# limix/CellRegMap

Hardware: AMD Instinct MI355X
Metric: variant-tests/sec (interaction test) (higher is better)
Workload: dtype f64

## Files before the change

### cellregmap_amd/csrc/api_core.hip

```cpp
#include <dlfcn.h>

#include <algorithm>
#include <atomic>
#include <cstdarg>
#include <mutex>

#include <map>

#include "crm_internal.h"
#include "eigh.h"

namespace crm {

static thread_local std::string g_error;

void set_error(const char* fmt, ...) {
    char buf[1024];
    va_list ap;
    va_start(ap, fmt);
    vsnprintf(buf, sizeof buf, fmt, ap);
    va_end(ap);
    g_error = buf;
}

// ... 235 lines not shown

int crm_set_null_fit_polish(crm_ctx* c, int on) {
    return crm::guarded_on("crm_set_null_fit_polish", c, [&]() -> int {
    if (!c) return CRM_ERR_ARG;
    c->polish = on != 0;
    return CRM_OK;
    });
}

int crm_set_progress_callback(crm_ctx* c, void (*callback)(long, long, void*), void* user) {
    return crm::guarded_on("crm_set_progress_callback", c, [&]() -> int {
    if (!c) return CRM_ERR_ARG;
    if (callback) c->progress[std::this_thread::get_id()] = crm_ctx::Progress{callback, user};
    else c->progress.erase(std::this_thread::get_id());
    return CRM_OK;
    });
}

int crm_set_fast_rotation(crm_ctx* c, int on) {
    return crm::guarded_on("crm_set_fast_rotation", c, [&]() -> int {
    if (!c) return CRM_ERR_ARG;
    c->fast_T = on != 0;
    return CRM_OK;
    });
}

extern "C++" {
namespace crm {
namespace {
struct FormSlot { const char* name; int value; bool set; };
FormSlot g_forms[] = {{"gram_staged", 0, false}, {"kr_no_tail", 0, false}, {"nullfit_per_wave", 0, false}, {"kin_fold", 0, false},
                      {"eigh_one_stage", 0, false}, {"nullfit_exact", 0, false}, {"donor_pairs", 0, false},
                      {"pairs_without_kinship_term", 0, false}, {"flat_kappa_milli", 0, false}, {"chase_abort", 0, false}, {"nullfit_one_per_wave", 0, false},
                      {"kin_diag", 0, false}, {"donor_pairs_rotate", 0, false}};
std::mutex g_forms_mu;
}
int form(const char* name, int otherwise) {
    std::lock_guard<std::mutex> lock(g_forms_mu);
    for (const FormSlot& f : g_forms)
        if (strcmp(f.name, name) == 0) return f.set ? f.value : otherwise;
    return otherwise;
}
}
}

int crm_test_set_form(const char* name, int value, int reset) {
    return crm::guarded("crm_test_set_form", [&]() -> int {
    if (!name) return CRM_ERR_ARG;
    std::lock_guard<std::mutex> lock(crm::g_forms_mu);
    for (crm::FormSlot& f : crm::g_forms)
        if (strcmp(f.name, name) == 0) {
            f.value = value;
            f.set = reset == 0;
            return CRM_OK;
        }
    crm::set_error("crm_test_set_form: no kernel form is called '%s'", name);
    return CRM_ERR_ARG;
    });
}

int crm_kernel_timer_reset(crm_ctx* c) {
    return crm::guarded_on("crm_kernel_timer_reset", c, [&]() -> int {
    if (!c) return CRM_ERR_ARG;
    CRM_HIP(hipSetDevice(c->device));
    CRM_HIP(hipStreamSynchronize(c->stream));
    c->timed_used = 0;
    c->kr_flops = 0.0;
// ... 270 lines not shown
```

### cellregmap_amd/csrc/blockops.hip

```cpp
#include "nullfit.h"

namespace crm {

namespace {

constexpr int STAT_SPLITS = 64;

__device__ __forceinline__ void row_and_chunk(int chunks, long& row, int& chunk) {
    row = blockIdx.x / (unsigned)chunks;
    chunk = (int)(blockIdx.x - (unsigned)row * (unsigned)chunks);
}
inline dim3 row_chunk_grid(long rows, int chunks) { return dim3((unsigned)(rows * chunks)); }

template <int C>
__global__ __launch_bounds__(256) void variant_stats_kernel(const double* __restrict__ G, long ldg,
                                                           long cells, int variants,
                                                           const double* __restrict__ y,
                                                           const double* __restrict__ W, long ldw,
                                                           double* __restrict__ partial) {
    __shared__ double red[4][C + 2][64];
    const int tx = threadIdx.x & 63, ty = threadIdx.x >> 6;
    const int b = blockIdx.x * 64 + tx;
    const long per = (cells + STAT_SPLITS - 1) / STAT_SPLITS;
    const long i0 = (long)blockIdx.y * per;
// ... 449 lines not shown
}

__global__ void pair_rows_sym_kernel(const double* __restrict__ C, long ldc, int variants, int k0, double* __restrict__ S,
                                     long lds) {
    const int a = blockIdx.y;
    const long e = (long)blockIdx.x * blockDim.x + threadIdx.x;
    if (e >= (long)variants * k0) return;
    const long b = e / k0;
    const int i = (int)(e - b * k0);
    const int lo = a < i ? a : i, hi = a < i ? i : a;
    const long pidx = (long)lo * k0 - (long)lo * (lo - 1) / 2 + (hi - lo);
    S[(long)a * lds + e] = C[b * ldc + pidx];
}

int launch_pair_rows_sym(hipStream_t st, const double* C, long ldc, int variants, int k0, double* S, long lds) {
    if (variants <= 0 || k0 <= 0) return CRM_OK;
    dim3 grid((unsigned)(((long)variants * k0 + 255) / 256), (unsigned)k0);
    hipLaunchKernelGGL(pair_rows_sym_kernel, grid, dim3(256), 0, st, C, ldc, variants, k0, S, lds);
    CRM_HIP(hipGetLastError());
    return CRM_OK;
}

constexpr int DP_VARIANTS = 4, DP_MAX_SLOTS = 32;

template <int DP_SLOTS>
__global__ __launch_bounds__(256) void donor_pairs_expand_kernel(const double* __restrict__ P, long p_slab, long ldp, int donors,
                                                                  int variants, int k0, int k1, double* __restrict__ S, long lds,
                                                                  double* __restrict__ Psum, long psum_slab, long row_d, long row_j) {
    extern __shared__ double tile[];
    const int npair = k0 * (k0 + 1) / 2, total = DP_VARIANTS * npair;
    const int v0 = blockIdx.x * DP_VARIANTS, tid = threadIdx.x;
    const int per = (donors + gridDim.y - 1) / gridDim.y;
    const int d0 = blockIdx.y * per, d1 = min(donors, d0 + per);
    if (d0 >= d1) return;
    double acc[DP_SLOTS], x[DP_SLOTS];
    int src[DP_SLOTS];
#pragma unroll
    for (int q = 0; q < DP_SLOTS; q++) {
        const int e = tid + 256 * q, v = e / npair, pr = e - v * npair;
        acc[q] = 0.0;
        src[q] = e < total && v0 + v < variants ? (int)((long)(v0 + v) * ldp + pr) : -1;
    }
    auto fetch = [&](int d) {
        const double* __restrict__ Pd = P + (size_t)d * p_slab;
#pragma unroll
        for (int q = 0; q < DP_SLOTS; q++)
            if (tid + 256 * q < total) x[q] = src[q] >= 0 ? Pd[src[q]] : 0.0;
    };
    const int row_len = DP_VARIANTS * k0;
    const int vw = tid / k0, iw = tid - vw * k0;
    const bool writer = tid < row_len && v0 + vw < variants;
    const int base_i = iw * k0 - iw * (iw - 1) / 2 - iw;
    const double* __restrict__ mine = tile + vw * npair;
    fetch(d0);
    for (int d = d0; d < d1; d++) {
#pragma unroll
        for (int q = 0; q < DP_SLOTS; q++)
            if (tid + 256 * q < total) { acc[q] += x[q]; tile[tid + 256 * q] = x[q]; }
        __syncthreads();
        if (d + 1 < d1) fetch(d + 1);
        if (writer) {
            double* __restrict__ Sd = S + (size_t)(k1 + (long)d * row_d) * lds + (long)v0 * k0 + tid;
            for (int j = 0; j < k0; j++) {
                const int pidx = j <= iw ? j * k0 - j * (j - 1) / 2 + (iw - j) : base_i + j;
                Sd[(long)j * row_j * lds] = mine[pidx];
            }
        }
// ... 1 lines not shown
    }
    double* __restrict__ out = Psum + (size_t)blockIdx.y * psum_slab;
#pragma unroll
    for (int q = 0; q < DP_SLOTS; q++)
        if (tid + 256 * q < total && src[q] >= 0) out[src[q]] = acc[q];
}

bool donor_pairs_serves(int k0) { return k0 >= 2 && DP_VARIANTS * (k0 * (k0 + 1) / 2) <= 256 * DP_MAX_SLOTS && DP_VARIANTS * k0 <= 256; }

int launch_donor_pairs_expand(hipStream_t st, const double* P, long p_slab, long ldp, int donors, int variants, int k0, int k1,
                              double* S, long lds, double* Psum, long psum_slab, int splits, long row_d, long row_j) {
    if (row_d <= 0) { row_d = k0; row_j = 1; }
    if (variants <= 0 || donors <= 0) return CRM_OK;
    if (!donor_pairs_serves(k0) || splits < 1) {
        set_error("donor pairs: k0=%d outside the supported range", k0);
        return CRM_ERR_UNSUPPORTED;
    }
    const size_t lds_bytes = sizeof(double) * DP_VARIANTS * (size_t)(k0 * (k0 + 1) / 2);
    dim3 grid((unsigned)((variants + DP_VARIANTS - 1) / DP_VARIANTS), (unsigned)splits);
    const int slots = (DP_VARIANTS * (k0 * (k0 + 1) / 2) + 255) / 256;
#define CRM_DP_LAUNCH(SL)                                                                                                        \
    hipLaunchKernelGGL(donor_pairs_expand_kernel<SL>, grid, dim3(256), lds_bytes, st, P, p_slab, ldp, donors, variants, k0, k1, \
                       S, lds, Psum, psum_slab, row_d, row_j)
    if (slots <= 4) CRM_DP_LAUNCH(4);
    else if (slots <= 8) CRM_DP_LAUNCH(8);
    else if (slots <= 16) CRM_DP_LAUNCH(16);
    else if (slots <= 24) CRM_DP_LAUNCH(24);
    else CRM_DP_LAUNCH(32);
#undef CRM_DP_LAUNCH
    CRM_HIP(hipGetLastError());
    return CRM_OK;
}

constexpr int DR_LDU = 80;
typedef double v4d __attribute__((ext_vector_type(4)));

__device__ __forceinline__ void lds_barrier() { asm volatile("s_waitcnt lgkmcnt(0)\n\ts_barrier" ::: "memory"); }

template <int DP_SLOTS>
__global__ __launch_bounds__(256, 2) void donor_pairs_rotate_kernel(const double* __restrict__ P, long p_slab, long ldp, int donors,
                                                                     int variants, int k0, const double* __restrict__ U, long u_slab,
                                                                     long ldu, double* __restrict__ A, long lda,
                                                                     double* __restrict__ Psum, long psum_slab) {
    extern __shared__ __align__(16) double smem[];
    const int npair = k0 * (k0 + 1) / 2, total = DP_VARIANTS * npair;
    const int KS = (k0 + 3) / 4, JT = (k0 + 15) / 16, urows = 4 * KS;
    double* const tile = smem;
    double* const ut = smem + ((total + 1) & ~1);
    const int v0 = blockIdx.x * DP_VARIANTS, tid = threadIdx.x;
    const int per = (donors + gridDim.y - 1) / gridDim.y;
    const int d0 = blockIdx.y * per, d1 = min(donors, d0 + per);
    if (d0 >= d1) return;
    double acc[DP_SLOTS];
#pragma unroll
    for (int q = 0; q < DP_SLOTS; q++) acc[q] = 0.0;
    const float inv_npair = 1.0f / (float)npair;
    const int vmax = min(DP_VARIANTS, variants - v0);
    auto src_of = [&](int q) __attribute__((always_inline)) -> int {
        int e = tid + 256 * q;
        asm volatile("" : "+v"(e));
        int v = (int)((float)e * inv_npair);
        v = v * npair > e ? v - 1 : ((v + 1) * npair <= e ? v + 1 : v);
        return e < total && v < vmax ? v * (int)ldp + (e - v * npair) : -1;
    };
    const int lane = tid & 63, l15 = lane & 15, lq = lane >> 4;
    const int w = __builtin_amdgcn_readfirstlane(tid >> 6);
    const int i = 16 * w + l15;
    int pidx[16];
#pragma unroll
    for (int ks = 0; ks < 16; ks++) {
        const int k = 4 * ks + lq, lo = k < i ? k : i, hi = k < i ? i : k;
        pidx[ks] = k < k0 && i < k0 ? lo * k0 - lo * (lo - 1) / 2 + (hi - lo) : 0;
    }
    for (int d = d0; d < d1; d++) {
        const double* __restrict__ Pd = P + (size_t)d * p_slab + (long)v0 * ldp;
#pragma unroll
        for (int q0 = 0; q0 < DP_SLOTS; q0 += 8) {
            double x[8];
            int sq[8];
#pragma unroll
            for (int q = 0; q < 8; q++) sq[q] = src_of(q0 + q);
#pragma unroll
            for (int q = 0; q < 8; q++) x[q] = Pd[sq[q] >= 0 ? sq[q] : 0];
#pragma unroll
            for (int q = 0; q < 8; q++)
                if (tid + 256 * (q0 + q) < total) {
                    const double xv = sq[q] >= 0 ? x[q] : 0.0;
                    acc[q0 + q] += xv;
                    tile[tid + 256 * (q0 + q)] = xv;
                }
        }
        const double* __restrict__ Ud = U + (size_t)d * u_slab + (tid & 63);
        double* __restrict__ ud = ut + (tid >> 6) * DR_LDU + (tid & 63);
#pragma unroll
        for (int q0 = 0; q0 < 16; q0 += 8) {
            double u[8];
#pragma unroll
            for (int q = 0; q < 8; q++) {
                int r = min((tid >> 6) + 4 * (q0 + q), urows - 1);
                asm volatile("" : "+v"(r));
                u[q] = Ud[(long)r * ldu];
            }
#pragma unroll
            for (int q = 0; q < 8; q++)
                if ((tid >> 6) + 4 * (q0 + q) < urows) ud[4 * (q0 + q) * DR_LDU] = u[q];
        }
        lds_barrier();
        if (w < JT) {
            for (int b = 0; b < DP_VARIANTS && v0 + b < variants; b++) {
                unsigned uo = (unsigned)(lq * DR_LDU + l15);
                asm volatile("" : "+v"(uo));
                const double* __restrict__ ub = ut + uo;
                const double* __restrict__ pb = tile + b * npair;
                v4d c[4];
#pragma unroll
                for (int t = 0; t < 4; t++) c[t] = (v4d){0.0, 0.0, 0.0, 0.0};
                double a[2], bf[2][4];
                auto frag = [&](int ks, int slot) __attribute__((always_inline)) {
                    a[slot] = pb[pidx[ks]];
#pragma unroll
                    for (int t = 0; t < 4; t++)
                        if (t < JT) bf[slot][t] = ub[4 * ks * DR_LDU + 16 * t];
                };
                frag(0, 0);
#pragma unroll
                for (int ks = 0; ks < 16; ks++) {
                    if (ks < KS) {
                        if (ks + 1 < KS) frag(ks + 1, (ks + 1) & 1);
#pragma unroll
                        for (int t = 0; t < 4; t++)
                            if (t < JT) c[t] = __builtin_amdgcn_mfma_f64_16x16x4f64(a[ks & 1], bf[ks & 1][t], c[t], 0, 0, 0);
                        __builtin_amdgcn_sched_barrier(0);
                    }
                }
                double* __restrict__ Ab = A + (size_t)((long)(v0 + b) * k0) * lda + (long)d * k0;
#pragma unroll
                for (int reg = 0; reg < 4; reg++) {
                    int r = 16 * w + lq + 4 * reg;
                    asm volatile("" : "+v"(r));
                    if (r < k0) {
#pragma unroll
                        for (int t = 0; t < 4; t++) {
                            const int j = 16 * t + l15;
                            if (t < JT && j < k0) Ab[(long)r * lda + j] = c[t][reg];
                        }
                    }
                }
            }
        }
        lds_barrier();
    }
    double* __restrict__ out = Psum + (size_t)blockIdx.y * psum_slab + (long)v0 * ldp;
#pragma unroll
    for (int q = 0; q < DP_SLOTS; q++) {
        const int sq = src_of(q);
        if (sq >= 0) out[sq] = acc[q];
    }
}

bool donor_pairs_rotate_serves(int k0) { return donor_pairs_serves(k0) && DP_VARIANTS * (k0 * (k0 + 1) / 2) <= 256 * 24; }

int launch_donor_pairs_rotate(hipStream_t st, const double* P, long p_slab, long ldp, int donors, int variants, int k0,
                              const double* U, long u_slab, long ldu, int k2pad, double* A, long lda, double* Psum, long psum_slab,
                              int splits) {
    if (variants <= 0 || donors <= 0) return CRM_OK;
    if (!donor_pairs_rotate_serves(k0) || splits < 1 || k2pad < 4 * ((k0 + 3) / 4) || ldu < 64) {
        set_error("donor pairs rotation: k0=%d / k2pad=%d outside the supported range", k0, k2pad);
        return CRM_ERR_UNSUPPORTED;
    }
    const int total = DP_VARIANTS * (k0 * (k0 + 1) / 2);
    const size_t lds_bytes = sizeof(double) * ((size_t)((total + 1) & ~1) + (size_t)4 * ((k0 + 3) / 4) * DR_LDU);
    dim3 grid((unsigned)((variants + DP_VARIANTS - 1) / DP_VARIANTS), (unsigned)splits);
    const int slots = (total + 255) / 256;
#define CRM_DR_LAUNCH(SL)                                                                                                         \
    do {                                                                                                                          \
        CRM_HIP(hipFuncSetAttribute(reinterpret_cast<const void*>(&donor_pairs_rotate_kernel<SL>),                                \
                                    hipFuncAttributeMaxDynamicSharedMemorySize, (int)lds_bytes));                                 \
        hipLaunchKernelGGL(donor_pairs_rotate_kernel<SL>, grid, dim3(256), lds_bytes, st, P, p_slab, ldp, donors, variants, k0, \
                           U, u_slab, ldu, A, lda, Psum, psum_slab);                                                              \
    } while (0)
    if (slots <= 8) CRM_DR_LAUNCH(8);
    else if (slots <= 16) CRM_DR_LAUNCH(16);
    else CRM_DR_LAUNCH(24);
#undef CRM_DR_LAUNCH
    CRM_HIP(hipGetLastError());
    return CRM_OK;
}

__global__ void scale_rows_kernel(const double* __restrict__ src, long ld_src, const double* __restrict__ scale, long ld_scale,
                                  int cols, double* __restrict__ dst, long ld_dst) {
    const long k = blockIdx.x;
    const double f = scale[k * ld_scale];
    for (int j = threadIdx.x; j < cols; j += blockDim.x) dst[k * ld_dst + j] = src[k * ld_src + j] * f;
}

int launch_scale_rows(hipStream_t st, const double* src, long ld_src, const double* scale, long ld_scale, long rows, int cols,
                      double* dst, long ld_dst) {
    if (rows <= 0 || cols <= 0) return CRM_OK;
    hipLaunchKernelGGL(scale_rows_kernel, dim3((unsigned)rows), dim3(128), 0, st, src, ld_src, scale, ld_scale, cols, dst, ld_dst);
    CRM_HIP(hipGetLastError());
    return CRM_OK;
}

__global__ void pair_rows_kernel(const double* __restrict__ C, long ldc, int variants, int k1, int k0,
                                 double* __restrict__ S, long lds) {
    const int a = blockIdx.y;
    const long e = (long)blockIdx.x * blockDim.x + threadIdx.x;
    if (e >= (long)variants * k0) return;
    const long b = e / k0;
    const int i = (int)(e - b * k0);
    S[(long)a * lds + e] = C[b * ldc + (long)a * k0 + i];
}

int launch_pair_rows(hipStream_t st, const double* C, long ldc, int variants, int k1, int k0, double* S, long lds) {
    if (variants <= 0 || k1 <= 0) return CRM_OK;
    dim3 grid((unsigned)(((long)variants * k0 + 255) / 256), (unsigned)k1);
// ... 64 lines not shown
```

### cellregmap_amd/csrc/nullfit.h

```cpp
#pragma once
#include "crm_internal.h"

namespace crm {

struct NullFitRho {
    const double* T;
    const double* ty;
    const double* tW;
    const double* S0;
    long ldT, ldW;
    int r;
    int pad_;
};

struct NullFitTrial {
    double lml, delta, scale;
    int use_g, nfev;
    double margin;
    double noise;
    double curv;
};

struct NullFitOut {
    int rho_index;
// ... 55 lines not shown
                         const double* y, const double* W, long ldw, int c, double* partial,
                         double* gg, double* gy, double* gW, long ld_gW);
size_t variant_stats_workspace(int variants, int c);
int launch_ortho_block(hipStream_t st, const double* G, long ldg, long cells_pad, int variants, int cols,
                       const double* W, long ldw, int c, const double* proj, const double* gW, long ld_gW,
                       double* coef, long ld_coef, double* thr, double* Gx, long ldx);
int launch_ortho_rank(hipStream_t st, const double* gg, const double* thr, int variants, int* drop);
int launch_collinear_flag(hipStream_t st, const double* gg, const double* gW, long ld_gW, const double* proj, int c,
                          int variants, double tau, int* near);
int launch_gather_block(hipStream_t st, const double* src, long ld_src, long cells_pad, long cells,
                        const int* row_index, const int* col_index, int variants, double* dst,
                        long ld_dst, int dst_cols);
int launch_gather_slabs(hipStream_t st, const double* src, long ld_src, long rows, const int* ord, int npairs,
                        int k0, double* dst, long ld_dst, int dst_cols);
int launch_gather_rows(hipStream_t st, const double* src, long ld_src, const int* map, long rows, int cols, double* dst,
                       long ld_dst);
int launch_kin_operand(hipStream_t st, const double* U, int k2, const double* H, long ldh, int k1, const int* map, long rows,
                       double* Y, long ldy);
int launch_kin_verify(hipStream_t st, const double* H, long ldh, int k1, const double* U, int k2, const int* group,
                      const double* hKd, long ldk, long m, long n, unsigned long long* out);
int launch_kin_sum_e1(hipStream_t st, const double* S, long ld_s, int KT, int k2, int k1, int groups, long cols, double* AH,
                      long ld_ah);
int launch_pair_features(hipStream_t st, const double* H, long ldh, int k1, const double* Ep, long ld_ep, int k0,
                         long cells_pad, double* P, long ldp);
int launch_pair_rows(hipStream_t st, const double* C, long ldc, int variants, int k1, int k0, double* S, long lds);
int launch_same_columns(hipStream_t st, const double* H, long ldh, const double* Ep, long ld_ep, long cells, int k, int* flag);
int launch_pair_rows_sym(hipStream_t st, const double* C, long ldc, int variants, int k0, double* S, long lds);
bool donor_pairs_serves(int k0);
int launch_donor_pairs_expand(hipStream_t st, const double* P, long p_slab, long ldp, int donors, int variants, int k0, int k1,
                              double* S, long lds, double* Psum, long psum_slab, int splits, long row_d = 0, long row_j = 0);
bool donor_pairs_rotate_serves(int k0);
int launch_donor_pairs_rotate(hipStream_t st, const double* P, long p_slab, long ldp, int donors, int variants, int k0,
                              const double* U, long u_slab, long ldu, int k2pad, double* A, long lda, double* Psum, long psum_slab,
                              int splits);
int launch_scale_rows(hipStream_t st, const double* src, long ld_src, const double* scale, long ld_scale, long rows, int cols,
                      double* dst, long ld_dst);
int launch_expand_block(hipStream_t st, const double* Gd, long ld_gd, const int* group, long cells_pad,
                        long cells, const int* row_index, int variants, double* dst, long ld_dst,
                        int dst_cols);
int launch_indicator(hipStream_t st, const int* group, long cells, long cells_pad, int m, double* Z, long ldz);
int launch_donor_stats(hipStream_t st, const double* Gam, long ld_gam, int m, int variants,
                       const double* sums, int c, double* gg, double* gy, double* gW, long ld_gW);
int launch_square_block(hipStream_t st, const double* Gt, const double* G, long ldg, long ldg_t,
                        long cells_pad, int cols, double* G2, double* GG, long ld_out);
int launch_context_features(hipStream_t st, const double* E, long lde, const int* row_index,
                            long cells, long cells_pad, int k0, const double* y, const double* W,
                            long ldw, int c, double* Ep, long ld_ep, double* YE, long ld_ye,
                            double* EE, long ld_ee);

struct AssembleRho {
    const double* ty;
    const double* tW;
    const double* S0;
    const double* T;
    long ldW, ldT;
    int r;
    int pad_;
    double rho;
};

struct AssembleArgs {
    AssembleRho rho[CRM_MAX_RHO];
    const NullFitOut* fit;
    const int* sorted_pos;
    const double* A;
    long ldA;
    const double* A_none;
// ... 33 lines not shown
```

### cellregmap_amd/csrc/scan.hip

```cpp
#include <algorithm>

#include "nullfit.h"
#include "objects.h"

using namespace crm;

namespace crm {

static int ctx_cus(const crm_ctx* ctx) {
    int cus = 256;
    if (hipDeviceGetAttribute(&cus, hipDeviceAttributeMultiprocessorCount, ctx->device) != hipSuccess || cus < 1) cus = 256;
    return cus;
}

constexpr double COLLINEAR_TAU = 1e-2;

__global__ void flat_probe_fit_kernel(const crm::NullFitOut* __restrict__ fit, int count, double sign,
                                      crm::NullFitOut* __restrict__ out) {
    const int b = blockIdx.x * blockDim.x + threadIdx.x;
    if (b >= count) return;
    crm::NullFitOut f = fit[b];
    const double tiny = 2.220446049250313e-16;
    const double d = fmin(fmax(f.delta, tiny), 1.0 - tiny);
    const double x = log(d) - log1p(-d);
// ... 35 lines not shown
    int* status = nullptr;
};

static bool scan_slow_forms(const crm_gene* g0) {
    return g0->k0 + g0->c + 2 > 144 || g0->k0 > 128 || assemble_rows_scratch_doubles(1, g0->k0, g0->c) > 0;
}
static int scan_block_variants(const crm_ctx* ctx, const crm_gene* g0, long count) {
    long auto_blk = (long)(16.0 * (1ull << 30) / (sizeof(double) * (double)g0->k0 * (double)g0->bg->ldq)) / 128 * 128;
    auto_blk = std::max<long>(256, std::min<long>(auto_blk, CRM_MAX_AUTO_BLOCK));
    int BLK = (int)std::min<long>(ctx->block_variants > 0 ? ctx->block_variants : auto_blk, round_up(count, 128));
    if (g0->c > CRM_MAX_COV_WIDE) BLK = std::min(BLK, 512);
    if (scan_slow_forms(g0)) BLK = std::min(BLK, 512);
    return BLK;
}

enum class Route {
    collapsed,
    direct,
    kin_unfolded,
    kin_folded,
    unrelated,
};

constexpr int SLOT_ONE = 0, SLOT_RHO = 1, SLOT_KIN = 2 * CRM_MAX_RHO + 4;

struct ScanPlan {
    Route route = Route::direct;
    bool fastT = false, slow_forms = false, skip_pairs = true, cross = false;
    bool e1_pairs = false, e1_sym = false, donor_pairs = false, wb_rotate = false, pairs_unfolded = false;
    int ng = 1, BLK = 0, pair_cap = 0;
    long ldb = 0, ldp = 0, ldA = 0, ldAw = 0, ldT = 0, ldZ1 = 0, ldZ2 = 0, ldZ3 = 0, ld_ah = 0, ld_xg = 0, ldP = 0, ldPd = 0,
         pd_slab = 0, ldwb = 0, ld_gW = 0, th_slab = 0, s_rows = 0;
    size_t s_bytes = 0;
    int ks1 = 1, ks2 = 1, ks3 = 1, ks_h = 1, fold_split6 = 1, fold_split3 = 1, donor_pair_splits = 1;
    int npair = 0, KT = 0, KK = 0, kin_probs = 0;
    long kdim = 0, mp = 0, xrows = 0;
    bool collapsed() const { return route == Route::collapsed; }
    bool kin() const { return route == Route::kin_unfolded || route == Route::kin_folded || route == Route::unrelated; }
    bool folded() const { return route == Route::kin_folded || route == Route::unrelated; }
    bool wb() const { return route == Route::unrelated; }
    bool through_H() const { return fastT && (ng > 1 || kin()); }
    int z1_slot() const { return SLOT_KIN + kin_probs; }
};

static double largest_rank(const crm_background* bg) {
    double rbar = 1.0;
    for (int i = 0; i < bg->nrho; i++) rbar = std::max(rbar, (double)bg->r[i]);
    return rbar;
}

static ScanPlan plan_scan(const std::vector<crm_gene*>& genes, const crm_panel* panel, const int* idx_G, bool allow_collapse,
                          long count) {
    const crm_gene* g0 = genes[0];
    const crm_background* bg = g0->bg;
    const crm_ctx* ctx = bg->ctx;
    const int ng = (int)genes.size(), nrho = bg->nrho, c = g0->c, k0 = g0->k0;
    const long n = bg->n, np = bg->n_pad, ldq = bg->ldq;
    ScanPlan P;
    P.ng = ng;
    P.slow_forms = scan_slow_forms(g0);
    const int BLK = P.BLK = scan_block_variants(ctx, g0, count);
    P.pair_cap = BLK;
    if (ng > 1) {
        const char* cap_env = getenv("CRM_PAIR_BUFFER_GB");
        const double cap_gb = cap_env && atof(cap_env) > 0 ? atof(cap_env) : 128.0;
        const double per_pair = 2.0 * sizeof(double) * k0 * (double)ldq;
        const long most = (long)std::min(nrho, ng) * BLK, least = (long)std::min(nrho, ng) * std::min(BLK, 128);
// ... 52 lines not shown
            : kin_route ? Route::kin_unfolded : Route::direct;
    P.ldAw = wb ? std::max<long>(P.ldA, bg->wb_ldp) : P.ldA;
    P.ldwb = wb ? bg->wb_ldp : 0;
    P.kdim = kfold ? bg->kin_kdim : bg->ldh;
    P.ldP = round_up((long)(bg->kin ? bg->kin_k1 : 0) * k0, 128);
    P.e1_pairs = kfold && sizeof(double) * (double)np * (double)P.ldP <= 8.0 * (1ull << 30);
    if (kfold) {
        const long tiles6 = P.e1_pairs ? ((long)BLK + GEMM_BM - 1) / GEMM_BM * (P.ldP / 128) : ((long)BLK * k0 + GEMM_BM - 1) / GEMM_BM;
        const long slots6 = P.e1_pairs || bg->kin_k1 > 64 ? 512 : 768;
        double best = 0.0;
        for (int sps = 1; sps <= 8 && np / GEMM_BK / sps >= 64; sps++) {
            const double rounds = (double)(tiles6 * sps) / (double)slots6, eff = rounds / std::ceil(rounds);
            if (eff > best + 0.02) { best = eff; P.fold_split6 = sps; }
        }
        const long tiles3 = (long)((bg->kin_k1 + GEMM_BM - 1) / GEMM_BM) * ((BLK + 127) / 128);
        while (tiles3 * P.fold_split3 < 1024 && P.fold_split3 < 16 && np / GEMM_BK / (P.fold_split3 + 1) >= 16) P.fold_split3++;
    }
    P.e1_sym = P.e1_pairs && bg->kin_k1 == k0;
    P.ldPd = round_up((long)P.npair, 128);
    P.pd_slab = (std::max<long>(BLK, max_pairs) + 128) * P.ldPd;
    if (P.e1_sym && bg->kin_k2 == k0 && donor_pairs_serves(k0) && form("donor_pairs", 1)) {
        const double peak = 78.6e12, hbm = 4.0e12;
        const double t_kr = 2.0 * bg->kin_rows * (double)k0 * k0 / (0.6 * peak) + 2.0 * (double)np * P.npair / (0.92 * peak);
        const double t_pairs = 2.0 * bg->kin_rows * (double)P.npair / (0.8 * peak) +
                               (double)bg->kin_groups * (2.0 * P.npair + (double)k0 * k0) * sizeof(double) / hbm;
        const bool fits = sizeof(double) * (double)bg->kin_groups * (double)P.pd_slab <= 8.0 * (1ull << 30);
        P.donor_pairs = fits && (t_pairs < t_kr || form("donor_pairs", 1) >= 2);
        const long wgs = (std::max<long>(BLK, 1) + 3) / 4;
        while ((wgs * P.donor_pair_splits) % 768 != 0 && wgs * P.donor_pair_splits < 4 * 768 && P.donor_pair_splits < 8 &&
               P.donor_pair_splits < bg->kin_groups)
            P.donor_pair_splits++;
    }
    P.wb_rotate = wb && P.donor_pairs && donor_pairs_rotate_serves(k0) && form("donor_pairs_rotate", 1) != 0;
    if (kin_route && !kfold && bg->kin_k1 == k0 && bg->kin_k2 == k0 && donor_pairs_serves(k0) && form("donor_pairs", 1) &&
        bg->kin_cols + 1 <= bg->kin_ldh) {
        const double cost_kr = 2.0 * bg->kin_rows * (double)P.KK * k0 + 2.0 * (double)bg->kin_groups_pad * bg->kin_cols * bg->kin_k2 * k0;
        const double cost_pairs = 2.0 * bg->kin_rows * (double)P.npair + 2.0 * (double)(bg->kin_cols + 1) * bg->kin_groups_pad * (double)P.ldPd;
        const bool fits = sizeof(double) * (double)bg->kin_groups_pad * (double)P.pd_slab <= 8.0 * (1ull << 30) &&
                          sizeof(double) * (double)(bg->kin_cols + 1) * (double)P.pd_slab <= (double)P.s_bytes;
        P.pairs_unfolded = fits && (cost_pairs < 0.8 * cost_kr || form("donor_pairs", 1) >= 2);
    }
    P.skip_pairs = form("pairs_without_kinship_term", 1) != 0;
    P.kin_probs = bg->kin ? bg->kin_groups * (bg->kin_wb ? 2 : 1) + bg->kin_k2 + 16 : 0;
    return P;
}

static long donor_run_records(const crm_background* bg, const GemmProblem& p, long c_step, GemmProblem* out) {
    long maxlen = GEMM_BK;
    for (long d = 0; d < bg->kin_groups; d++) {
        const long r0 = bg->kin_row0[d];
        GemmProblem q = p;
        q.X = p.X + r0 * p.ldx;
        if (p.E) q.E = p.E + r0 * p.lde;
        q.Y = p.Y + r0 * p.ldy; q.C = p.C + d * c_step; q.cells = bg->kin_len[d];
        maxlen = std::max(maxlen, bg->kin_len[d]);
        out[d] = q;
    }
    return maxlen;
}

static void woodbury_records(const crm_background* bg, const GemmProblem& p, long x_step, GemmProblem* out) {
    for (long d = 0; d < bg->kin_groups; d++) {
        GemmProblem q = p;
        q.X = p.X + d * x_step; q.Y = bg->wb_U.as<double>() + (size_t)d * bg->wb_k2pad * 128; q.ldy = 128;
        q.C = p.C + d * bg->kin_k2; q.N = bg->kin_k2; q.cells = bg->wb_k2pad;
        out[d] = q;
// ... 845 lines not shown
            p.E = g0->kinEp.as<double>(); p.lde = g0->ld_ep; p.k0 = k0; p.Y = bg->kin_Y.as<double>(); p.ldy = bg->kin_ldy;
            p.C = S + (size_t)k1 * ld_ah; p.ldc = ld_ah; p.M = ncol * k0; p.N = k2;
        }
        const long maxlen = donor_run_records(bg, p, P.donor_pairs ? P.pd_slab : (long)k2 * ld_ah, kp.data());
        const long stages_all = np / GEMM_BK, per = (stages_all + P.fold_split6 - 1) / P.fold_split6;
        const long e1_slab = (long)k1 * ld_ah;
        int slices = 0;
        long chunk_max = GEMM_BK;
        if (P.e1_pairs) {
            GemmProblem& e = kp[groups];
            e.X = D.G; e.ldx = D.ldg; e.Y = g0->kinP.as<double>(); e.ldy = P.ldP;
            e.C = ctx->ws_AH.as<double>(); e.ldc = P.ldP; e.M = ncol; e.N = k1 * k0;
            if (P.e1_sym) { e.Y = d_EE; e.ldy = g0->ld_ee; e.N = npair; }
        }
        for (int sps = 0; sps < P.fold_split6 && !P.e1_pairs; sps++) {
            const long s0 = sps * per, s1 = std::min(stages_all, s0 + per);
            if (s1 <= s0) break;
            GemmProblem& e = kp[groups + slices++];
            e.X = D.G + s0 * GEMM_BK * D.ldg; e.ldx = D.ldg;
            e.E = d_Ep + s0 * GEMM_BK * g0->ld_ep; e.lde = g0->ld_ep; e.k0 = k0;
            e.Y = bg->H.as<double>() + s0 * GEMM_BK * bg->ldh; e.ldy = bg->ldh;
            e.C = ctx->ws_AH.as<double>() + (size_t)sps * e1_slab; e.ldc = ld_ah;
            e.M = ncol * k0; e.N = k1; e.cells = (s1 - s0) * GEMM_BK;
            chunk_max = std::max(chunk_max, e.cells);
        }
        kp.resize((size_t)groups + std::max(slices, 1));
        return with_records(SLOT_KIN, kp, [&](GemmProblem* d_kp) -> int {
            double* AH = ctx->ws_AH.as<double>();
            if (P.donor_pairs) {
                CRM_TRY(launch_gemm_tn(ctx, d_kp, (int)groups, ncol, npair, maxlen, false, 0, 1, 0));
                if (P.wb_rotate)
                    CRM_TRY(launch_donor_pairs_rotate(st, ctx->ws_Pd.as<double>(), P.pd_slab, P.ldPd, (int)groups, ncol, k0,
                                                      bg->wb_U.as<double>(), (long)bg->wb_k2pad * 128, 128, bg->wb_k2pad,
                                                      ctx->ws_A.as<double>(), P.ldAw, AH, P.pd_slab, P.donor_pair_splits));
                else
                    CRM_TRY(launch_donor_pairs_expand(st, ctx->ws_Pd.as<double>(), P.pd_slab, P.ldPd, (int)groups, ncol, k0, k1, S, ld_ah,
                                                      AH, P.pd_slab, P.donor_pair_splits));
                CRM_TRY(launch_reduce_splits(st, AH, (long)ncol * P.ldPd, P.donor_pair_splits, P.pd_slab));
                CRM_TRY(launch_pair_rows_sym(st, AH, P.ldPd, ncol, k0, S, ld_ah));
                ctx->donor_pair_blocks++;
            } else {
                if (k2 == 1) CRM_TRY(launch_gemm_tn(ctx, d_kp, (int)groups, ncol, k0, maxlen, false, 0, 1, 0));
                else CRM_TRY(launch_kr_transposed(ctx, d_kp, (int)groups, ncol * k0, k2, maxlen, k0));
                if (P.e1_pairs) {
                    const long p_slab = (long)(std::max<long>(P.BLK, P.pair_cap) + 128) * P.ldP;
                    CRM_TRY(launch_gemm_tn(ctx, d_kp + groups, 1, ncol, P.e1_sym ? npair : k1 * k0, np, false, 0, P.fold_split6, p_slab));
                    CRM_TRY(launch_reduce_splits(st, AH, (long)ncol * P.ldP, P.fold_split6, p_slab));
                    if (P.e1_sym) CRM_TRY(launch_pair_rows_sym(st, AH, P.ldP, ncol, k0, S, ld_ah));
                    else CRM_TRY(launch_pair_rows(st, AH, P.ldP, ncol, k1, k0, S, ld_ah));
                } else {
                    CRM_TRY(launch_kr_transposed(ctx, d_kp + groups, slices, ncol * k0, k1, chunk_max, k0));
                    CRM_TRY(launch_reduce_splits(st, AH, e1_slab, slices, e1_slab));
                    CRM_HIP(hipMemcpyAsync(S, AH, sizeof(double) * (size_t)e1_slab, hipMemcpyDeviceToDevice, st));
                }
            }
            if (!D.in_pair_order && !P.wb()) CRM_TRY(gather_pairs(S, P.kdim, Q));
            return CRM_OK;
        });
    }

    int unfolded_AH(const Block& B, const SubRange& R, const Pairs& Q) {
        DonorCols D;
        CRM_TRY(donor_columns(B, R, Q, D));
        double* S = ctx->ws_S.as<double>();
        double* AH = ctx->ws_AH.as<double>();
        const int k1 = bg->kin_k1, k2 = bg->kin_k2, ncol = D.ncol, npair = P.npair;
        const long groups = bg->kin_groups, mk = bg->kin_cols, KK = P.KK, ld_ah = P.ld_ah;
// ... 643 lines not shown
```

Baseline: 70480.

## Warp-specialize donor pair rotation with async LDS double-buffered loads

Rewrites the donor-pair rotation kernel so dedicated loader waves stream each donor's pair tile and U rows into LDS with 16-byte global_load_lds DMA into a double buffer. Those loader waves also accumulate the per-donor pair sums, while eight compute waves run the matrix-core rotation on the current buffer. It separates the number of summation ranges from the grid split, so fewer workgroups can cover many donors, and zero-fills partial-sum slabs that no workgroup writes. The goal is to hide global load latency behind compute and to cut per-donor scalar load and store work. The cost is a larger LDS footprint, a new 16-byte alignment requirement on operands, and higher kernel complexity.

```diff
diff --git a/cellregmap_amd/csrc/api_core.hip b/cellregmap_amd/csrc/api_core.hip
--- a/cellregmap_amd/csrc/api_core.hip
+++ b/cellregmap_amd/csrc/api_core.hip
@@ -291,7 +291,8 @@
 FormSlot g_forms[] = {{"gram_staged", 0, false}, {"kr_no_tail", 0, false}, {"nullfit_per_wave", 0, false}, {"kin_fold", 0, false},
                       {"eigh_one_stage", 0, false}, {"nullfit_exact", 0, false}, {"donor_pairs", 0, false},
                       {"pairs_without_kinship_term", 0, false}, {"flat_kappa_milli", 0, false}, {"chase_abort", 0, false}, {"nullfit_one_per_wave", 0, false},
-                      {"kin_diag", 0, false}, {"donor_pairs_rotate", 0, false}};
+                      {"kin_diag", 0, false}, {"donor_pairs_rotate", 0, false}, {"donor_rotate_splits", 0, false},
+                      {"donor_pair_splits", 0, false}};
 std::mutex g_forms_mu;
 }
 int form(const char* name, int otherwise) {
diff --git a/cellregmap_amd/csrc/blockops.hip b/cellregmap_amd/csrc/blockops.hip
--- a/cellregmap_amd/csrc/blockops.hip
+++ b/cellregmap_amd/csrc/blockops.hip
@@ -505,7 +505,13 @@
     const int v0 = blockIdx.x * DP_VARIANTS, tid = threadIdx.x;
     const int per = (donors + gridDim.y - 1) / gridDim.y;
     const int d0 = blockIdx.y * per, d1 = min(donors, d0 + per);
-    if (d0 >= d1) return;
+    if (d0 >= d1) {
+        for (int e = tid; e < total; e += 256) {
+            const int v = e / npair;
+            if (v0 + v < variants) Psum[(size_t)blockIdx.y * psum_slab + (long)(v0 + v) * ldp + (e - v * npair)] = 0.0;
+        }
+        return;
+    }
     double acc[DP_SLOTS], x[DP_SLOTS];
     int src[DP_SLOTS];
 #pragma unroll
@@ -573,39 +579,108 @@
     return CRM_OK;
 }
 
-constexpr int DR_LDU = 80;
+constexpr int DR_COMPUTE_WAVES = 8, DR_LOAD_WAVES = 4, DR_THREADS = 64 * (DR_COMPUTE_WAVES + DR_LOAD_WAVES);
+constexpr int DR_LOADERS = 64 * DR_LOAD_WAVES;
+constexpr int DR_PQ = 12, DR_UQ = 8;
 typedef double v4d __attribute__((ext_vector_type(4)));
+typedef const double __attribute__((address_space(1))) * dr_gptr_t;
+typedef __attribute__((address_space(3))) void* dr_lptr_t;
 
 __device__ __forceinline__ void lds_barrier() { asm volatile("s_waitcnt lgkmcnt(0)\n\ts_barrier" ::: "memory"); }
 
-template <int DP_SLOTS>
-__global__ __launch_bounds__(256, 2) void donor_pairs_rotate_kernel(const double* __restrict__ P, long p_slab, long ldp, int donors,
-                                                                     int variants, int k0, const double* __restrict__ U, long u_slab,
-                                                                     long ldu, double* __restrict__ A, long lda,
-                                                                     double* __restrict__ Psum, long psum_slab) {
+__device__ __forceinline__ void dr_dma16(const double* src, double* lds_wave_uniform) {
+    __builtin_amdgcn_global_load_lds((dr_gptr_t)src, (dr_lptr_t)lds_wave_uniform, 16, 0, 0);
+}
+
+__host__ __device__ inline int dr_tile_doubles(int k0) {
+    const int np2 = (k0 * (k0 + 1) / 2 + 1) & ~1;
+    return 128 * ((DP_VARIANTS * (np2 / 2) + 63) / 64);
+}
+__host__ __device__ inline int dr_buffer_doubles(int k0) { return dr_tile_doubles(k0) + ((k0 + 3) / 4) * 4 * 64; }
+
+template <int DP_ROWQ>
+__global__ __launch_bounds__(DR_THREADS) void donor_pairs_rotate_kernel(const double* __restrict__ P, long p_slab, long ldp, int donors,
+                                                                        int variants, int k0, const double* __restrict__ U, long u_slab,
+                                                                        long ldu, double* __restrict__ A, long lda,
+                                                                        double* __restrict__ Psum, long psum_slab, int sum_ranges) {
     extern __shared__ __align__(16) double smem[];
-    const int npair = k0 * (k0 + 1) / 2, total = DP_VARIANTS * npair;
-    const int KS = (k0 + 3) / 4, JT = (k0 + 15) / 16, urows = 4 * KS;
-    double* const tile = smem;
-    double* const ut = smem + ((total + 1) & ~1);
+    const int npair = k0 * (k0 + 1) / 2, total = DP_VARIANTS * npair, np2 = (npair + 1) & ~1, hp = np2 / 2;
+    const int KS = (k0 + 3) / 4, JT = (k0 + 15) / 16;
+    const int tile_len = dr_tile_doubles(k0), buf_len = dr_buffer_doubles(k0);
     const int v0 = blockIdx.x * DP_VARIANTS, tid = threadIdx.x;
-    const int per = (donors + gridDim.y - 1) / gridDim.y;
-    const int d0 = blockIdx.y * per, d1 = min(donors, d0 + per);
+    const int sum_per = (donors + sum_ranges - 1) / sum_ranges, rpw = (sum_ranges + gridDim.y - 1) / gridDim.y;
+    const int r0 = blockIdx.y * rpw, r1 = min(sum_ranges, r0 + rpw);
+    const int d0 = min(donors, r0 * sum_per), d1 = min(donors, r1 * sum_per);
+    const int vmax = min(DP_VARIANTS, variants - v0);
+    for (int r = r0 + (d1 - d0 + sum_per - 1) / sum_per; r < r1; r++) {
+        double* __restrict__ zr = Psum + (size_t)r * psum_slab + (long)v0 * ldp;
+        for (int e = tid; e < total; e += DR_THREADS) {
+            const int v = e / npair;
+            if (v < vmax) zr[v * (int)ldp + (e - v * npair)] = 0.0;
+        }
+    }
     if (d0 >= d1) return;
-    double acc[DP_SLOTS];
-#pragma unroll
-    for (int q = 0; q < DP_SLOTS; q++) acc[q] = 0.0;
-    const float inv_npair = 1.0f / (float)npair;
-    const int vmax = min(DP_VARIANTS, variants - v0);
-    auto src_of = [&](int q) __attribute__((always_inline)) -> int {
-        int e = tid + 256 * q;
-        asm volatile("" : "+v"(e));
-        int v = (int)((float)e * inv_npair);
-        v = v * npair > e ? v - 1 : ((v + 1) * npair <= e ? v + 1 : v);
-        return e < total && v < vmax ? v * (int)ldp + (e - v * npair) : -1;
-    };
-    const int lane = tid & 63, l15 = lane & 15, lq = lane >> 4;
-    const int w = __builtin_amdgcn_readfirstlane(tid >> 6);
+    const int wave = __builtin_amdgcn_readfirstlane(tid >> 6), lane = tid & 63;
+
+    if (wave >= DR_COMPUTE_WAVES) {
+        const int lw = wave - DR_COMPUTE_WAVES, lt = tid - 64 * DR_COMPUTE_WAVES;
+        double acc[DP_VARIANTS][DP_ROWQ];
+#pragma unroll
+        for (int v = 0; v < DP_VARIANTS; v++)
+#pragma unroll
+            for (int q = 0; q < DP_ROWQ; q++) acc[v][q] = 0.0;
+        const int NI = tile_len / 128;
+        unsigned poff[DR_PQ];
+#pragma unroll
+        for (int q = 0; q < DR_PQ; q++) {
+            const int p = 64 * (lw + DR_LOAD_WAVES * q) + lane, v = p / hp, c = p - v * hp;
+            poff[q] = v < vmax ? (unsigned)(v * (int)ldp + 2 * c) : (v < DP_VARIANTS ? (unsigned)(2 * c) : 0u);
+        }
+        const long uoff = (long)(lane >> 5) * ldu + ((2 * (lane & 31)) ^ ((lane >> 5) << 4));
+        auto issue = [&](int d, double* buf) __attribute__((always_inline)) {
+            const double* __restrict__ Pd = P + (size_t)d * p_slab + (long)v0 * ldp;
+#pragma unroll
+            for (int q = 0; q < DR_PQ; q++) {
+                const int n = lw + DR_LOAD_WAVES * q;
+                if (n < NI) dr_dma16(Pd + poff[q], buf + n * 128);
+            }
+            const double* __restrict__ Ud = U + (size_t)d * u_slab + uoff;
+#pragma unroll
+            for (int q = 0; q < DR_UQ; q++) {
+                const int n = lw + DR_LOAD_WAVES * q;
+                if (n < 2 * KS) dr_dma16(Ud + (long)(2 * n) * ldu, buf + tile_len + n * 128);
+            }
+        };
+        issue(d0, smem);
+        asm volatile("s_waitcnt vmcnt(0)" ::: "memory");
+        lds_barrier();
+        for (int d = d0; d < d1; d++) {
+            const int s = (d - d0) & 1;
+            const double* __restrict__ cur = smem + s * buf_len;
+            if (d + 1 < d1) issue(d + 1, smem + (s ^ 1) * buf_len);
+#pragma unroll
+            for (int v = 0; v < DP_VARIANTS; v++)
+#pragma unroll
+                for (int q = 0; q < DP_ROWQ; q++)
+                    if (v < vmax && lt + DR_LOADERS * q < npair) acc[v][q] += cur[v * np2 + lt + DR_LOADERS * q];
+            if ((d + 1) % sum_per == 0 || d + 1 == d1) {
+                double* __restrict__ out = Psum + (size_t)(d / sum_per) * psum_slab + (long)v0 * ldp;
+#pragma unroll
+                for (int v = 0; v < DP_VARIANTS; v++)
+#pragma unroll
+                    for (int q = 0; q < DP_ROWQ; q++) {
+                        if (v < vmax && lt + DR_LOADERS * q < npair) out[v * ldp + lt + DR_LOADERS * q] = acc[v][q];
+                        acc[v][q] = 0.0;
+                    }
+            }
+            asm volatile("s_waitcnt vmcnt(0)" ::: "memory");
+            lds_barrier();
+        }
+        return;
+    }
+
+    const int l15 = lane & 15, lq = lane >> 4;
+    const int w = wave & 3, b0 = 2 * (wave >> 2);
     const int i = 16 * w + l15;
     int pidx[16];
 #pragma unroll
@@ -613,46 +688,18 @@
         const int k = 4 * ks + lq, lo = k < i ? k : i, hi = k < i ? i : k;
         pidx[ks] = k < k0 && i < k0 ? lo * k0 - lo * (lo - 1) / 2 + (hi - lo) : 0;
     }
+    const unsigned u_even = (unsigned)(lq * 64 + l15 + ((lq & 1) ? 16 : 0)), u_odd = (unsigned)(lq * 64 + l15 + ((lq & 1) ? 0 : 16));
+    lds_barrier();
     for (int d = d0; d < d1; d++) {
-        const double* __restrict__ Pd = P + (size_t)d * p_slab + (long)v0 * ldp;
-#pragma unroll
-        for (int q0 = 0; q0 < DP_SLOTS; q0 += 8) {
-            double x[8];
-            int sq[8];
-#pragma unroll
-            for (int q = 0; q < 8; q++) sq[q] = src_of(q0 + q);
-#pragma unroll
-            for (int q = 0; q < 8; q++) x[q] = Pd[sq[q] >= 0 ? sq[q] : 0];
-#pragma unroll
-            for (int q = 0; q < 8; q++)
-                if (tid + 256 * (q0 + q) < total) {
-                    const double xv = sq[q] >= 0 ? x[q] : 0.0;
-                    acc[q0 + q] += xv;
-                    tile[tid + 256 * (q0 + q)] = xv;
-                }
-        }
-        const double* __restrict__ Ud = U + (size_t)d * u_slab + (tid & 63);
-        double* __restrict__ ud = ut + (tid >> 6) * DR_LDU + (tid & 63);
-#pragma unroll
-        for (int q0 = 0; q0 < 16; q0 += 8) {
-            double u[8];
-#pragma unroll
-            for (int q = 0; q < 8; q++) {
-                int r = min((tid >> 6) + 4 * (q0 + q), urows - 1);
-                asm volatile("" : "+v"(r));
-                u[q] = Ud[(long)r * ldu];
-            }
-#pragma unroll
-            for (int q = 0; q < 8; q++)
-                if ((tid >> 6) + 4 * (q0 + q) < urows) ud[4 * (q0 + q) * DR_LDU] = u[q];
-        }
-        lds_barrier();
+        const double* __restrict__ cur = smem + ((d - d0) & 1) * buf_len;
         if (w < JT) {
-            for (int b = 0; b < DP_VARIANTS && v0 + b < variants; b++) {
-                unsigned uo = (unsigned)(lq * DR_LDU + l15);
-                asm volatile("" : "+v"(uo));
-                const double* __restrict__ ub = ut + uo;
-                const double* __restrict__ pb = tile + b * npair;
+            for (int bb = 0; bb < 2 && v0 + b0 + bb < variants; bb++) {
+                const int b = b0 + bb;
+                unsigned ue = u_even, uo = u_odd;
+                asm volatile("" : "+v"(ue), "+v"(uo));
+                const double* __restrict__ ube = cur + tile_len + ue;
+                const double* __restrict__ ubo = cur + tile_len + uo;
+                const double* __restrict__ pb = cur + b * np2;
                 v4d c[4];
 #pragma unroll
                 for (int t = 0; t < 4; t++) c[t] = (v4d){0.0, 0.0, 0.0, 0.0};
@@ -661,7 +708,7 @@
                     a[slot] = pb[pidx[ks]];
 #pragma unroll
                     for (int t = 0; t < 4; t++)
-                        if (t < JT) bf[slot][t] = ub[4 * ks * DR_LDU + 16 * t];
+                        if (t < JT) bf[slot][t] = ((t & 1) ? ubo : ube)[4 * ks * 64 + 32 * (t >> 1)];
                 };
                 frag(0, 0);
 #pragma unroll
@@ -691,38 +738,40 @@
         }
         lds_barrier();
     }
-    double* __restrict__ out = Psum + (size_t)blockIdx.y * psum_slab + (long)v0 * ldp;
-#pragma unroll
-    for (int q = 0; q < DP_SLOTS; q++) {
-        const int sq = src_of(q);
-        if (sq >= 0) out[sq] = acc[q];
-    }
-}
-
-bool donor_pairs_rotate_serves(int k0) { return donor_pairs_serves(k0) && DP_VARIANTS * (k0 * (k0 + 1) / 2) <= 256 * 24; }
+}
+
+bool donor_pairs_rotate_serves(int k0) {
+    return donor_pairs_serves(k0) && k0 * (k0 + 1) / 2 <= DR_LOADERS * 6 &&
+           dr_tile_doubles(k0) / 128 <= DR_LOAD_WAVES * DR_PQ && 2 * ((k0 + 3) / 4) <= DR_LOAD_WAVES * DR_UQ &&
+           sizeof(double) * 2 * (size_t)dr_buffer_doubles(k0) <= 160 * 1024;
+}
 
 int launch_donor_pairs_rotate(hipStream_t st, const double* P, long p_slab, long ldp, int donors, int variants, int k0,
                               const double* U, long u_slab, long ldu, int k2pad, double* A, long lda, double* Psum, long psum_slab,
-                              int splits) {
+                              int sum_ranges, int splits) {
     if (variants <= 0 || donors <= 0) return CRM_OK;
-    if (!donor_pairs_rotate_serves(k0) || splits < 1 || k2pad < 4 * ((k0 + 3) / 4) || ldu < 64) {
+    if (!donor_pairs_rotate_serves(k0) || splits < 1 || splits > 65535 || sum_ranges < splits || k2pad < 4 * ((k0 + 3) / 4) || ldu < 64) {
         set_error("donor pairs rotation: k0=%d / k2pad=%d outside the supported range", k0, k2pad);
         return CRM_ERR_UNSUPPORTED;
     }
-    const int total = DP_VARIANTS * (k0 * (k0 + 1) / 2);
-    const size_t lds_bytes = sizeof(double) * ((size_t)((total + 1) & ~1) + (size_t)4 * ((k0 + 3) / 4) * DR_LDU);
+    const int npair = k0 * (k0 + 1) / 2;
+    if (((uintptr_t)P | (uintptr_t)U) % 16 != 0 || (p_slab | ldp | u_slab | ldu) % 2 != 0 || ldp < ((npair + 1) & ~1)) {
+        set_error("donor pairs rotation: operands not laid out for 16-byte loads (ldp=%ld, ldu=%ld)", ldp, ldu);
+        return CRM_ERR_UNSUPPORTED;
+    }
+    const size_t lds_bytes = sizeof(double) * 2 * (size_t)dr_buffer_doubles(k0);
     dim3 grid((unsigned)((variants + DP_VARIANTS - 1) / DP_VARIANTS), (unsigned)splits);
-    const int slots = (total + 255) / 256;
-#define CRM_DR_LAUNCH(SL)                                                                                                         \
+    const int rowq = (npair + DR_LOADERS - 1) / DR_LOADERS;
+#define CRM_DR_LAUNCH(RQ)                                                                                                         \
     do {                                                                                                                          \
-        CRM_HIP(hipFuncSetAttribute(reinterpret_cast<const void*>(&donor_pairs_rotate_kernel<SL>),                                \
+        CRM_HIP(hipFuncSetAttribute(reinterpret_cast<const void*>(&donor_pairs_rotate_kernel<RQ>),                                \
                                     hipFuncAttributeMaxDynamicSharedMemorySize, (int)lds_bytes));                                 \
-        hipLaunchKernelGGL(donor_pairs_rotate_kernel<SL>, grid, dim3(256), lds_bytes, st, P, p_slab, ldp, donors, variants, k0, \
-                           U, u_slab, ldu, A, lda, Psum, psum_slab);                                                              \
+        hipLaunchKernelGGL(donor_pairs_rotate_kernel<RQ>, grid, dim3(DR_THREADS), lds_bytes, st, P, p_slab, ldp, donors, variants, \
+                           k0, U, u_slab, ldu, A, lda, Psum, psum_slab, sum_ranges);                                              \
     } while (0)
-    if (slots <= 8) CRM_DR_LAUNCH(8);
-    else if (slots <= 16) CRM_DR_LAUNCH(16);
-    else CRM_DR_LAUNCH(24);
+    if (rowq <= 2) CRM_DR_LAUNCH(2);
+    else if (rowq <= 4) CRM_DR_LAUNCH(4);
+    else CRM_DR_LAUNCH(6);
 #undef CRM_DR_LAUNCH
     CRM_HIP(hipGetLastError());
     return CRM_OK;
diff --git a/cellregmap_amd/csrc/nullfit.h b/cellregmap_amd/csrc/nullfit.h
--- a/cellregmap_amd/csrc/nullfit.h
+++ b/cellregmap_amd/csrc/nullfit.h
@@ -111,7 +111,7 @@
 bool donor_pairs_rotate_serves(int k0);
 int launch_donor_pairs_rotate(hipStream_t st, const double* P, long p_slab, long ldp, int donors, int variants, int k0,
                               const double* U, long u_slab, long ldu, int k2pad, double* A, long lda, double* Psum, long psum_slab,
-                              int splits);
+                              int sum_ranges, int splits);
 int launch_scale_rows(hipStream_t st, const double* src, long ld_src, const double* scale, long ld_scale, long rows, int cols,
                       double* dst, long ld_dst);
 int launch_expand_block(hipStream_t st, const double* Gd, long ld_gd, const int* group, long cells_pad,
diff --git a/cellregmap_amd/csrc/scan.hip b/cellregmap_amd/csrc/scan.hip
--- a/cellregmap_amd/csrc/scan.hip
+++ b/cellregmap_amd/csrc/scan.hip
@@ -91,7 +91,7 @@
     long ldb = 0, ldp = 0, ldA = 0, ldAw = 0, ldT = 0, ldZ1 = 0, ldZ2 = 0, ldZ3 = 0, ld_ah = 0, ld_xg = 0, ldP = 0, ldPd = 0,
          pd_slab = 0, ldwb = 0, ld_gW = 0, th_slab = 0, s_rows = 0;
     size_t s_bytes = 0;
-    int ks1 = 1, ks2 = 1, ks3 = 1, ks_h = 1, fold_split6 = 1, fold_split3 = 1, donor_pair_splits = 1;
+    int ks1 = 1, ks2 = 1, ks3 = 1, ks_h = 1, fold_split6 = 1, fold_split3 = 1, donor_pair_splits = 1, donor_rotate_splits = 1;
     int npair = 0, KT = 0, KK = 0, kin_probs = 0;
     long kdim = 0, mp = 0, xrows = 0;
     bool collapsed() const { return route == Route::collapsed; }
@@ -210,6 +210,12 @@
             P.donor_pair_splits++;
     }
     P.wb_rotate = wb && P.donor_pairs && donor_pairs_rotate_serves(k0) && form("donor_pairs_rotate", 1) != 0;
+    if (P.donor_pairs && form("donor_pair_splits", 0) >= 1) P.donor_pair_splits = std::min(form("donor_pair_splits", 0), 65535);
+    if (P.wb_rotate) {
+        const long wgs = (std::max<long>(BLK, 1) + 3) / 4;
+        while (wgs * P.donor_rotate_splits < 256 && P.donor_rotate_splits < P.donor_pair_splits) P.donor_rotate_splits++;
+        if (form("donor_rotate_splits", 0) >= 1) P.donor_rotate_splits = std::min(form("donor_rotate_splits", 0), P.donor_pair_splits);
+    }
     if (kin_route && !kfold && bg->kin_k1 == k0 && bg->kin_k2 == k0 && donor_pairs_serves(k0) && form("donor_pairs", 1) &&
         bg->kin_cols + 1 <= bg->kin_ldh) {
         const double cost_kr = 2.0 * bg->kin_rows * (double)P.KK * k0 + 2.0 * (double)bg->kin_groups_pad * bg->kin_cols * bg->kin_k2 * k0;
@@ -1121,7 +1127,8 @@
                 if (P.wb_rotate)
                     CRM_TRY(launch_donor_pairs_rotate(st, ctx->ws_Pd.as<double>(), P.pd_slab, P.ldPd, (int)groups, ncol, k0,
                                                       bg->wb_U.as<double>(), (long)bg->wb_k2pad * 128, 128, bg->wb_k2pad,
-                                                      ctx->ws_A.as<double>(), P.ldAw, AH, P.pd_slab, P.donor_pair_splits));
+                                                      ctx->ws_A.as<double>(), P.ldAw, AH, P.pd_slab, P.donor_pair_splits,
+                                                      P.donor_rotate_splits));
                 else
                     CRM_TRY(launch_donor_pairs_expand(st, ctx->ws_Pd.as<double>(), P.pd_slab, P.ldPd, (int)groups, ncol, k0, k1, S, ld_ah,
                                                       AH, P.pd_slab, P.donor_pair_splits));
```

After: 72200 (median of 6 runs). +2.4%, better.
